# bigai-nlco/VideoTGB

Hardware: AMD Instinct MI355X
Metric: clips/sec end-to-end VideoQA (96->8 frames) (higher is better)
Workload: dtype bf16; 1 GPU; InstructBLIP-Vicuna-7B + TGB, T=96->8 of 32 frames, 224x224, greedy 16 new tokens (BASELINE.json configs[2]); inputs=resident in HBM when the timed region starts, global_batch=124, parallelism=clip-parallel x1 (no data-path collective), streams=1, weights=seeded N(0,0.02) random init

## Files before the change

include/vtgb.h:

```cpp
#ifndef VTGB_H
#define VTGB_H

#include <stddef.h>
#include <stdint.h>

#ifdef __cplusplus
extern "C" {
#endif

typedef struct ihipStream_t* vtgb_stream_t;

#define VTGB_VERSION 601

#define VTGB_OK 0
#define VTGB_EINVAL (-1)
#define VTGB_EWORKSPACE (-2)
#define VTGB_EHIP (-3)
#define VTGB_EUNSUPPORTED (-4)

#define VTGB_F32 0
#define VTGB_BF16 1
#define VTGB_BF16X3 2
#define VTGB_F16C8 3

// ... 239 lines not shown
typedef struct {
    int32_t M, N, H, W, KH, KW, C1;
    const void* a;
    const void* a2;
    const void* weights;
    const int32_t* scale;
    const float* bias;
    int32_t act;
    int32_t out_fmt;
    void* out;
    int32_t ld_out;
} vtgb_pair_conv_args;
int vtgb_pair_conv(const vtgb_pair_conv_args* a, vtgb_stream_t stream);
typedef struct {
    vtgb_pair_conv_args conv;
    const void* resid;
    int32_t ld_resid;
    const float* tail_w;
    float* tail_out;
    float* out_f32;
    int32_t ld_f32;
} vtgb_pair_conv_ex_args;
int vtgb_pair_conv_ex(const vtgb_pair_conv_ex_args* a, vtgb_stream_t stream);

typedef struct {
    int32_t dtype, n_pairs, H8, W8, dim;
    int32_t pairs_per_clip, frames_per_clip, first_off, second_off, n_images;
    float scale;
    const float* fmap;
    void* levels[4];
    void* workspace;
    size_t workspace_bytes;
} vtgb_raft_corr_args;
size_t vtgb_raft_corr_workspace_bytes(const vtgb_raft_corr_args* a);
int vtgb_raft_corr(const vtgb_raft_corr_args* a, vtgb_stream_t stream);

#define VTGB_RAFT_ENC_NW 40
typedef struct {
    int32_t dtype, n_images, H, W, norm;
    const float* images;
    const void* const* weights;
    float* out;
    void* workspace;
    size_t workspace_bytes;
} vtgb_raft_encoder_args;
size_t vtgb_raft_encoder_workspace_bytes(const vtgb_raft_encoder_args* a);
// ... 153 lines not shown
```

videotgb_amd/_lib.py:

```python
from __future__ import annotations

import ctypes as C
import os

import torch

HERE = os.path.dirname(os.path.abspath(__file__))
LIB_PATH = os.environ.get("VTGB_LIB") or os.path.join(HERE, "libvtgb.so")

F32, BF16 = 0, 1
BF16X3 = 2
F16C8 = 3
MAP_A, MAP_B = 0, 1
POOL_MEAN, POOL_CONCAT = 0, 1
TGB_MODE = {"text": 0, "vision": 0, "fusion": 1, "multi_modal": 2}
EPI_STORE, EPI_GELU, EPI_RESID_F32, EPI_STORE_F32 = 0, 1, 2, 3
VIT_NW_GLOBAL, VIT_NW_LAYER = 6, 18
QF_NW_GLOBAL, QF_NW_LAYER = 4, 32
TGB_NW_GLOBAL, TGB_NW_LAYER = 17, 26

EXPORTS = [
    "vtgb_version", "vtgb_last_error", "vtgb_pack_bf16", "vtgb_span_select", "vtgb_span_to_frames",
    "vtgb_gather_frames", "vtgb_vit_patch_kpad", "vtgb_vit_workspace_bytes", "vtgb_vit_forward",
    "vtgb_qformer_workspace_bytes", "vtgb_qformer_forward", "vtgb_pool_project_workspace_bytes",
    "vtgb_pool_project", "vtgb_tgb_workspace_bytes", "vtgb_tgb_forward", "vtgb_tgb_trunk_workspace_bytes", "vtgb_tgb_trunk",
    "vtgb_tgb_resume_workspace_bytes", "vtgb_tgb_resume", "vtgb_gemm", "vtgb_attention",
    "vtgb_layernorm", "vtgb_prof_enable", "vtgb_prof_reset", "vtgb_prof_summary", "vtgb_prof_executed_flops",
    "vtgb_llm_rmsnorm", "vtgb_llm_rope_cache", "vtgb_llm_rope_cache_prefill", "vtgb_llm_decode_attention", "vtgb_llm_silu_mul",
    "vtgb_llm_attention_rows", "vtgb_llm_gated_act", "vtgb_llm_rmsnorm_parts", "vtgb_llm_rope_cache_parts", "vtgb_gemm_skinny_splits",
    "vtgb_llm_rope_cache_pos", "vtgb_llm_rope_cache_parts_pos", "vtgb_llm_rope_cache_prefill_pos", "vtgb_llm_decode_attention_masked",
    "vtgb_llm_attention_rows_masked",
    "vtgb_gemm_skinny_workspace_bytes", "vtgb_gemm_skinny", "vtgb_pack_skinny_weight_bytes", "vtgb_pack_skinny_weight",
    "vtgb_pack_skinny_weight_fp8_bytes", "vtgb_pack_skinny_weight_fp8", "vtgb_gemm_skinny_fp8",
    "vtgb_raft_update_workspace_bytes", "vtgb_raft_update", "vtgb_raft_encoder_workspace_bytes", "vtgb_raft_encoder",
    "vtgb_raft_corr_workspace_bytes", "vtgb_raft_corr", "vtgb_preprocess_frames", "vtgb_concat_text_io", "vtgb_shifted_ce_forward", "vtgb_shifted_ce_backward",
    "vtgb_comm_unique_id", "vtgb_comm_init", "vtgb_comm_destroy", "vtgb_allreduce_f32",
    "vtgb_attn_train_forward", "vtgb_attn_train_backward",
    "vtgb_gemm_train", "vtgb_gemm_train_workspace_bytes", "vtgb_col_sum_parts", "vtgb_col_sum_f32", "vtgb_layernorm_train_partials", "vtgb_layernorm_train_forward", "vtgb_layernorm_train_backward",
    "vtgb_gelu_forward", "vtgb_gelu_backward",
    "vtgb_pair_pack", "vtgb_pair_conv", "vtgb_pair_conv_ex", "vtgb_attention_tiled",
    "vtgb_llm_decode_attention_split_workspace_bytes", "vtgb_llm_decode_attention_split",
]
COMM_ID_BYTES = 128

i32, i64, f32, vp, sz = C.c_int32, C.c_int64, C.c_float, C.c_void_p, C.c_size_t


class AttnTrainArgs(C.Structure):
    _fields_ = [("batch", i32), ("heads", i32), ("head_dim", i32), ("s_q", i32), ("s_kv", i32), ("q", vp), ("k", vp), ("v", vp),
                ("q_tok", i64), ("kv_tok", i64), ("q_batch", i64), ("kv_batch", i64), ("key_mask", vp), ("drop", vp), ("scale", f32),
                ("out", vp), ("o_tok", i64), ("o_batch", i64), ("lse", vp), ("dout", vp), ("dq", vp), ("dk", vp), ("dv", vp), ("delta", vp)]


class GemmTrainArgs(C.Structure):
    _fields_ = [("compute", i32), ("M", i32), ("N", i32), ("K", i32), ("a", vp), ("lda", i64), ("a_dtype", i32), ("a_kmajor", i32),
                ("b", vp), ("ldb", i64), ("b_dtype", i32), ("b_kmajor", i32), ("bias", vp), ("out", vp), ("ldo", i64), ("workspace", vp), ("workspace_bytes", sz)]


class LayerNormTrainArgs(C.Structure):
    _fields_ = [("rows", i32), ("D", i32), ("eps", f32), ("x", vp), ("mask", vp), ("resid", vp), ("gamma", vp), ("beta", vp), ("sum", vp),
                ("y", vp), ("mean", vp), ("rstd", vp), ("dy", vp), ("ds", vp), ("dx", vp), ("dgamma", vp), ("dbeta", vp), ("partial", vp)]


# ... 143 lines not shown
    L.vtgb_vit_patch_kpad.restype = i32
    for name, st in (("span_select", SpanSelectArgs), ("span_to_frames", SpanToFramesArgs),
                     ("gather_frames", GatherFramesArgs), ("vit_forward", VitArgs), ("qformer_forward", QFormerArgs),
                     ("pool_project", PoolProjectArgs), ("tgb_forward", TgbArgs), ("gemm", GemmArgs),
                     ("attention", AttentionArgs), ("attention_tiled", AttentionTiledArgs), ("layernorm", LayerNormArgs)):
        fn = getattr(L, "vtgb_" + name)
        fn.argtypes = [C.POINTER(st), vp]
        fn.restype = C.c_int
    for name, st in (("vit", VitArgs), ("qformer", QFormerArgs), ("pool_project", PoolProjectArgs), ("tgb", TgbArgs),
                     ("tgb_trunk", TgbSplitArgs), ("tgb_resume", TgbSplitArgs)):
        fn = getattr(L, f"vtgb_{name}_workspace_bytes")
        fn.argtypes = [C.POINTER(st)]
        fn.restype = sz
    for name in ("tgb_trunk", "tgb_resume"):
        fn = getattr(L, "vtgb_" + name)
        fn.argtypes = [C.POINTER(TgbSplitArgs), vp]
        fn.restype = C.c_int
    L.vtgb_pair_pack.argtypes = [i32, vp, vp, i64, i32, i32, vp]
    L.vtgb_pair_pack.restype = C.c_int
    L.vtgb_pair_conv.argtypes = [C.POINTER(PairConvArgs), vp]
    L.vtgb_pair_conv.restype = C.c_int
    L.vtgb_pair_conv_ex.argtypes = [C.POINTER(PairConvExArgs), vp]
    L.vtgb_pair_conv_ex.restype = C.c_int
    L.vtgb_raft_update.argtypes = [C.POINTER(RaftUpdateArgs), vp]
    L.vtgb_raft_update.restype = C.c_int
    L.vtgb_raft_update_workspace_bytes.argtypes = [C.POINTER(RaftUpdateArgs)]
    L.vtgb_raft_update_workspace_bytes.restype = sz
    L.vtgb_raft_encoder.argtypes = [C.POINTER(RaftEncoderArgs), vp]
    L.vtgb_raft_encoder.restype = C.c_int
    L.vtgb_raft_encoder_workspace_bytes.argtypes = [C.POINTER(RaftEncoderArgs)]
    L.vtgb_raft_encoder_workspace_bytes.restype = sz
    L.vtgb_raft_corr.argtypes = [C.POINTER(RaftCorrArgs), vp]
    L.vtgb_raft_corr.restype = C.c_int
    L.vtgb_raft_corr_workspace_bytes.argtypes = [C.POINTER(RaftCorrArgs)]
    L.vtgb_raft_corr_workspace_bytes.restype = sz
    L.vtgb_llm_rmsnorm.argtypes = [C.c_int, vp, vp, vp, vp, i64, i32, f32, vp]
    L.vtgb_llm_rope_cache.argtypes = [C.c_int, vp, vp, vp, vp, vp, vp, vp, i32, i32, i32, i32, i32, vp]
    L.vtgb_llm_rope_cache_prefill.argtypes = [C.c_int, vp, vp, vp, vp, vp, i32, i32, i32, i32, i32, i32, vp]
    L.vtgb_llm_decode_attention.argtypes = [C.c_int, vp, vp, vp, vp, vp, i32, i32, i32, i32, i32, f32, vp]
    L.vtgb_llm_silu_mul.argtypes = [C.c_int, vp, vp, i64, i32, vp]
    L.vtgb_llm_attention_rows.argtypes = [C.POINTER(LlmAttnRowsArgs), vp]
    L.vtgb_llm_attention_rows.restype = C.c_int
    L.vtgb_llm_gated_act.argtypes = [C.c_int, vp, vp, i64, i32, i32, i32, vp]
    L.vtgb_llm_gated_act.restype = C.c_int
    L.vtgb_llm_rmsnorm_parts.argtypes = [C.c_int, vp, vp, i32, vp, vp, i64, i32, f32, vp]
    L.vtgb_llm_rmsnorm_parts.restype = C.c_int
# ... 85 lines not shown
```

videotgb_amd/build.py:

```python
import os
import subprocess
import sys

HERE = os.path.dirname(os.path.abspath(__file__))
REPO = os.path.dirname(HERE)
CSRC = os.path.join(HERE, "csrc")
LIB = os.path.join(HERE, "libvtgb.so")
SOURCES = ["gemm.hip", "gemm_pp.hip", "gemm_h8.hip", "conv64.hip", "conv_f32.hip", "attn.hip", "attn_tiled.hip", "attn_decode.hip", "elementwise.hip", "select.hip", "forward.hip", "llm.hip", "gemm_skinny.hip", "raft.hip", "raft_x3.hip", "gru_fused.hip", "raft_corr.hip", "raft_enc.hip", "train.hip", "train_attn.hip", "train_ops.hip", "comm.hip"]


FLAGS_STAMP = os.path.join(HERE, "build", "flags")


def _flags():
    return ("debug-hooks" if os.environ.get("VTGB_DEBUG_HOOKS") == "1" else "production") + os.environ.get("VTGB_CFLAGS", "")


def _stale():
    if not os.path.exists(LIB):
        return True
    if not os.path.exists(FLAGS_STAMP) or open(FLAGS_STAMP).read() != _flags():
        return True
    t = os.path.getmtime(LIB)
    deps = [os.path.join(CSRC, f) for f in os.listdir(CSRC)] + [os.path.join(REPO, "include", "vtgb.h")]
    return any(os.path.getmtime(d) > t for d in deps)


def build(force: bool = False, verbose: bool = False) -> str:
    if not force and not _stale():
        return LIB
    hipcc = os.environ.get("HIPCC", "/opt/rocm/bin/hipcc")
# ... 31 lines not shown
```

videotgb_amd/csrc/common.h:

```cpp
#pragma once
#include <hip/hip_runtime.h>
#include <stdint.h>
#include <stdio.h>

#include "vtgb.h"

typedef __bf16 bf16_t;
typedef __attribute__((ext_vector_type(8))) __bf16 bf16x8;
typedef __attribute__((ext_vector_type(4))) __bf16 bf16x4;
typedef __attribute__((ext_vector_type(4))) float f32x4;

#if defined(__HIPCC__)
__device__ __forceinline__ float bf16_round(float v) {
    unsigned u = __float_as_uint(v);
    if ((u & 0x7F800000u) != 0x7F800000u) u += 0x7FFFu + ((u >> 16) & 1u);
    return __uint_as_float(u & 0xFFFF0000u);
}
#endif

void vtgb_set_error(const char* fmt, ...);

#define VTGB_REQUIRE(cond, code, ...)  \
    do {                               \
        if (!(cond)) {                 \
// ... 134 lines not shown
    const void *q, *k, *v;
    int64_t q_tok, kv_tok, q_batch, kv_batch;
    const float* key_mask;
    const float* rope_q;
    const float* rope_k;
    float scale;
    void* out;
    int64_t o_tok, o_batch;
    int causal = 0;
};
int launch_attention(const AttnDesc& d, hipStream_t s);

bool stem7x7_supported(int H, int W);
int launch_stem7x7(const float* img, const void* w, const float* bias, float* out_f32, float* stats, float* stats_part, void* out_bf16, int n_img, int H, int W,
                   int relu, hipStream_t s);
size_t conv64_stats_part_floats(int n_img);
int launch_stats_finish_tiles(const float* part, float* stats, int n_img, int HW, int N, int64_t M, hipStream_t s);
int launch_stats_finish_parts(const float* part, float* stats, int n_img, int parts, int C, hipStream_t s);
int cu_count();

bool conv3x3_c64_supported(int H, int W);
int launch_conv3x3_c64(const void* in, const void* w, const float* bias, float* out_f32, float* stats, float* stats_part, void* out_bf16, const void* resid,
                       int n_img, int H, int W, int relu, int post_relu, hipStream_t s);

struct LnDesc {
    int dtype, M, D;
    float eps;
    const float* x;
    int64_t ldx;
    RowMap x_map;
    const float* gamma;
    const float* beta;
    float* out_f32;
    void* out_act;
    int64_t ldo;
    RowMap o_map;
};
int launch_layernorm(const LnDesc& d, hipStream_t s);

int launch_im2col(int dtype, const float* pix, void* out, int n_img, int ch, int image, int patch, int kpad, hipStream_t s);
int launch_vit_cls_rows(const float* cls, const float* pos, float* x, int n_frames, int tokens, int hidden, hipStream_t s);
int launch_cast_act(int dtype, const float* src, void* dst, int64_t n, hipStream_t s);
int launch_mask_to_additive(const int64_t* mask, float* out, int64_t n, float neg, hipStream_t s);
int launch_fill_f32(float* dst, float v, int64_t n, hipStream_t s);
int launch_qformer_embed(const float* query, const int64_t* ids, const float* wemb, const float* pemb, float* x,
                         int n_frames, int n_query, int n_text, int hidden, hipStream_t s);
// ... 19 lines not shown
```

videotgb_amd/csrc/raft_enc.hip:

```cpp
#include <math.h>
#include <string.h>

#include "common.h"

template <typename T>
__global__ __launch_bounds__(256) void raft_stem_pack_kernel(const float* __restrict__ img, T* __restrict__ out, T* __restrict__ pad_page,
                                                             int64_t n_px, int H, int W) {
    constexpr bool PAIR = sizeof(T) == 2;
    constexpr int CP = PAIR ? 128 : 64;
    const int64_t i = (int64_t)blockIdx.x * blockDim.x + threadIdx.x;
    if (i < 64) pad_page[i] = (T)0.f;
    if (i >= n_px * 4) return;
    const int64_t px_i = i >> 2;
    const int dX = (int)(i & 3), W2 = W >> 1, H2 = H >> 1;
    const int X = (int)(px_i % W2), Y = (int)((px_i / W2) % H2);
    const int64_t n = px_i / ((int64_t)W2 * H2);
    T v[12], l[12];
#pragma unroll
    for (int py = 0; py < 2; py++)
#pragma unroll
        for (int pxx = 0; pxx < 2; pxx++) {
            const int col = 2 * (X + dX - 2) + pxx, row = 2 * Y + py;
            const bool ok = (unsigned)col < (unsigned)W;
#pragma unroll
// ... 320 lines not shown
                memset(&d, 0, sizeof(d));
                d.dtype = VTGB_BF16; d.M = (int)Mo; d.N = g.C; d.K = 9 * C2; d.epi = VTGB_EPI_STORE_F32;
                d.A = A; d.lda = C2; d.W = Wt; d.ldw = d.K; d.bias = bias; d.out = cf; d.ldo = g.Cpad;
                d.conv_H = g.Ho; d.conv_W = g.Wo; d.conv_KH = 3; d.conv_KW = 3; d.conv_Cin = C2; d.conv_split = C2; d.zero_page = zero;
                d.col_stats = col_stats; d.stats_rows = HWo;
                d.h8_run = 9 * (g.Cpad / 64); d.h8_scale = (const int*)w[40] + si;
                d.algo_flops = 2.0 * Mo * (double)g.C * (9 * g.C);
                VTGB_TRY(launch_conv_h8(d, s));
                if (col_stats) VTGB_TRY(launch_stats_finish_tiles(col_stats, stats, n, HWo, g.C, Mo, s));
                return VTGB_OK;
            };
            auto conv_pair = [&](const void* A, const void* Wt, const float* bias, int si, const void* resid, void* out, int out_bf16) -> int {
                GemmDesc d;
                memset(&d, 0, sizeof(d));
                d.dtype = VTGB_BF16; d.M = (int)Mo; d.N = g.Cpad; d.K = 9 * C2; d.epi = VTGB_EPI_SPLIT; d.act = 1;
                d.A = A; d.lda = C2; d.W = Wt; d.ldw = d.K; d.bias = bias; d.out = out; d.ldo = C2; d.split_lo = g.Cpad;
                d.conv_H = g.Ho; d.conv_W = g.Wo; d.conv_KH = 3; d.conv_KW = 3; d.conv_Cin = C2; d.conv_split = C2; d.zero_page = zero;
                d.resid_bf16 = resid; d.ldrb = C2; d.post_relu = resid != nullptr;
                d.h8_run = 9 * (g.Cpad / 64); d.h8_scale = (const int*)w[40] + si; d.h8_out_bf16 = out_bf16;
                d.algo_flops = 2.0 * Mo * (double)g.C * (9 * g.C);
                return launch_conv_h8(d, s);
            };
            const int out_h8 = (b & 1) == 0;
            if (!inorm) {
                auto split_conv = [&](int K, const void* Wt, const float* bias, int relu, void* out) -> int {
                    GemmDesc d = enc_conv(dt, (int)Mo, g.Cpad, g.Ho, g.Wo, K, Cin_pad, g.stride, Hi, Wi, x, Wt, bias, nullptr, C2, zero, nullptr);
                    d.epi = VTGB_EPI_SPLIT; d.act = relu; d.out = out; d.split_lo = g.Cpad; d.split_f16c8 = 1;
                    d.algo_flops = 2.0 * Mo * (double)g.C * (K * K * Cin_pad);
                    return launch_conv_gemm(d, s);
                };
                if (s2) VTGB_TRY(split_conv(3, bw[0], F(bw[1]), 1, t1));
                else VTGB_TRY(conv_pair(x, bw[0], F(bw[1]), 2 * b, nullptr, t1, 0));
                const void* res = x;
                outb = t2;
                if (s2) {
                    VTGB_TRY(split_conv(1, bw[4], F(bw[5]), 0, t2));
                    res = t2;
                    outb = x;
                }
                VTGB_TRY(conv_pair(t1, bw[2], F(bw[3]), 2 * b + 1, res, outb, !out_h8));
            } else {
                float* sf = stats_for(stats, HWo, g.C);
                if (s2) VTGB_TRY(conv_stats(enc_conv(dt, (int)Mo, g.C, g.Ho, g.Wo, 3, Cin_pad, g.stride, Hi, Wi, x, bw[0], F(bw[1]), cf, g.Cpad, zero, sf), stats));
                else VTGB_TRY(conv_h8(x, bw[0], F(bw[1]), sf, 2 * b));
                VTGB_TRY(norm(cf, Mo, HWo, g.C, g.Cpad, g.Cpad, nullptr, t1, 1, 0, stats, sf != nullptr, 1));
                sf = stats_for(stats, HWo, g.C);
                VTGB_TRY(conv_h8(t1, bw[2], F(bw[3]), sf, 2 * b + 1));
                const void* res = x;
                if (s2) {
                    float* sf2 = stats_for(stats2, HWo, g.C);
                    VTGB_TRY(conv_stats(enc_conv(dt, (int)Mo, g.C, g.Ho, g.Wo, 1, Cin_pad, g.stride, Hi, Wi, x, bw[4], F(bw[5]), cf2, g.Cpad, zero, sf2), stats2));
                    VTGB_TRY(norm(cf2, Mo, HWo, g.C, g.Cpad, g.Cpad, nullptr, t2, 0, 0, stats2, sf2 != nullptr));
                    res = t2;
                }
                outb = t1;
                VTGB_TRY(norm(cf, Mo, HWo, g.C, g.Cpad, g.Cpad, res, outb, 1, 1, stats, sf != nullptr, out_h8, !s2));
            }
        } else if (x3 && !inorm && g.Cpad == 128) {
            auto split_conv = [&](int K, int Cin, int stride, int Hi_, int Wi_, const void* A, const void* Wt, const float* bias, int relu, void* out) -> int {
                GemmDesc d = enc_conv(dt, (int)Mo, g.Cpad, g.Ho, g.Wo, K, Cin, stride, Hi_, Wi_, A, Wt, bias, nullptr, 2 * g.Cpad, zero, nullptr);
                d.epi = VTGB_EPI_SPLIT; d.act = relu; d.out = out; d.split_lo = g.Cpad;
                d.algo_flops = 2.0 * Mo * (double)g.C * (K * K * Cin);
                return launch_conv_gemm(d, s);
// ... 55 lines not shown
```

videotgb_amd/csrc/raft_x3.hip:

```cpp
#include <math.h>
#include <string.h>

#include "common.h"
#include "pair_h8.h"

int raft_launch_lookup_pair(const CorrPyr& pyr, const float* flow, void* out_pair, int64_t M, int H8, int W8, int h8, hipStream_t s);
int raft_lkc1_h8_pack(const void* w, void* packed, hipStream_t s);
size_t raft_lkc1_h8_pack_bytes();
int raft_launch_lookup_convc1_h8(const CorrPyr& pyr, const float* flow, const void* wpk, const int* scale, const float* bias, void* c1, int64_t M, int H8, int W8,
                                 hipStream_t s);
int raft_launch_flow_head2(const float* P2, const float* bias, float* flow, int n_pairs, int H8, int W8, hipStream_t s);
int raft_launch_upsample(const float* flow, const float* mask, float* flow_up, int n_pairs, int H8, int W8, hipStream_t s);

__device__ __forceinline__ void pair_split4(const f32x4 v, bf16x4& hi, bf16x4& lo) {
#pragma unroll
    for (int e = 0; e < 4; e++) {
        const float hf = bf16_round(v[e]);
        hi[e] = (bf16_t)hf;
        lo[e] = (bf16_t)(v[e] - hf);
    }
}
__device__ __forceinline__ f32x4 pair_join4(const bf16x4 hi, const bf16x4 lo) {
    return f32x4{(float)hi[0] + (float)lo[0], (float)hi[1] + (float)lo[1], (float)hi[2] + (float)lo[2], (float)hi[3] + (float)lo[3]};
}
// ... 341 lines not shown
        }
        if (h8) {
            GemmDesc fh = conv(256, 3, 3, hb, 128, nullptr, 0, 18, 7, F(w[19]), VTGB_EPI_SPLIT, 1, FH, 512, 256, 1);
            fh.tail_w = w[20]; fh.tail_out = P2; fh.ldtail = 32;
            VTGB_TRY(run(fh));
        } else {
            VTGB_TRY(run(conv(256, 3, 3, hb, 128, nullptr, 0, 18, 7, F(w[19]), VTGB_EPI_SPLIT, 1, FH, 512, 256, 1)));
            VTGB_TRY(launch_conv_gemm(x3_conv(Mi, 32, H8, W8, 1, 1, FH, 256, nullptr, 0, w[20], nullptr, VTGB_EPI_STORE_F32, 0, P2, 32, 0, zero), s));
        }
        VTGB_TRY(raft_launch_flow_head2(P2, F(w[21]), flow, a->n_pairs, H8, W8, s));
    }
    VTGB_TRY(run(conv(256, 3, 3, hb, 128, nullptr, 0, 22, 8, F(w[23]), VTGB_EPI_SPLIT, 1, FH, 512, 256, 1)));
    VTGB_TRY(launch_conv_gemm(x3_conv(Mi, 576, H8, W8, 1, 1, FH, 256, nullptr, 0, w[24], F(w[25]), VTGB_EPI_STORE_F32, 0, mask, 576, 0, zero), s));
    VTGB_TRY(raft_launch_upsample(flow, mask, a->flow_up, a->n_pairs, H8, W8, s));
    VTGB_HIP(hipGetLastError());
    return VTGB_OK;
}

extern "C" int vtgb_pair_pack(int32_t fmt, const float* x, void* out, int64_t M, int32_t C, int32_t ld_pair, vtgb_stream_t stream) {
    VTGB_REQUIRE(x && out && M > 0 && C > 0 && (C & 3) == 0 && ld_pair >= C && (ld_pair & 3) == 0 && (fmt == VTGB_F16C8 || fmt == VTGB_BF16X3), VTGB_EINVAL,
                 "pair_pack: bad argument (C=%d ld_pair=%d fmt=%d)", C, ld_pair, fmt);
    return launch_x3_pair_pass(x, C, nullptr, 1, nullptr, 0, 0, out, 2 * (int64_t)ld_pair, ld_pair, C, ld_pair, 0, 0, M, (hipStream_t)stream, fmt == VTGB_F16C8, 0);
}
static int pair_conv_impl(const vtgb_pair_conv_args* a, const vtgb_pair_conv_ex_args* x, vtgb_stream_t stream);
extern "C" int vtgb_pair_conv(const vtgb_pair_conv_args* a, vtgb_stream_t stream) { return pair_conv_impl(a, nullptr, stream); }
extern "C" int vtgb_pair_conv_ex(const vtgb_pair_conv_ex_args* x, vtgb_stream_t stream) {
    VTGB_REQUIRE(x, VTGB_EINVAL, "pair_conv_ex: NULL args");
    VTGB_REQUIRE((x->resid != nullptr) + (x->tail_w != nullptr) + (x->out_f32 != nullptr) <= 1, VTGB_EINVAL, "pair_conv_ex: at most one of resid / tail_w / out_f32");
    return pair_conv_impl(&x->conv, x, stream);
}
static int pair_conv_impl(const vtgb_pair_conv_args* a, const vtgb_pair_conv_ex_args* x, vtgb_stream_t stream) {
    VTGB_REQUIRE(a && a->a && a->weights && a->scale && a->out && a->M > 0 && a->N > 0 && (a->N & 1) == 0 && a->C1 > 0 && (a->C1 % 64) == 0 && a->ld_out >= a->N &&
                     (a->ld_out & 3) == 0 && (a->out_fmt == VTGB_F16C8 || a->out_fmt == VTGB_BF16X3) && (a->act == 0 || a->act == 1),
                 VTGB_EINVAL, "pair_conv: bad argument");
    static void* zero = nullptr;
    if (!zero) {
        VTGB_HIP(hipMalloc(&zero, 256));
        VTGB_HIP(hipMemset(zero, 0, 256));
    }
    GemmDesc d = h8_conv(a->M, a->N, a->H, a->W, a->KH, a->KW, a->a, a->C1, a->a2, a->a2 ? a->C1 : 0, a->weights, a->bias, VTGB_EPI_SPLIT, a->act, a->out, 2 * (int64_t)a->ld_out,
                         a->ld_out, zero, a->scale, a->out_fmt == VTGB_BF16X3);
    if (x && x->resid) {
        VTGB_REQUIRE(x->ld_resid >= a->N && (x->ld_resid & 3) == 0 && x->ld_resid == a->ld_out, VTGB_EINVAL, "pair_conv_ex: the skip operand's pair rows have the output's layout");
        d.resid_bf16 = x->resid; d.ldrb = 2 * (int64_t)x->ld_resid; d.post_relu = 1;
    }
    if (x && x->tail_w) {
        VTGB_REQUIRE(x->tail_out, VTGB_EINVAL, "pair_conv_ex: tail_out is NULL");
        d.tail_w = x->tail_w; d.tail_out = x->tail_out; d.ldtail = 32;
    }
    if (x && x->out_f32) {
        VTGB_REQUIRE(x->ld_f32 >= a->N && (x->ld_f32 & 3) == 0, VTGB_EINVAL, "pair_conv_ex: fp32 rows need ld_f32 >= N, %% 4 == 0");
        d.epi = VTGB_EPI_STORE_F32; d.out = x->out_f32; d.ldo = x->ld_f32; d.split_lo = 0;
    }
    return launch_conv_h8(d, (hipStream_t)stream);
}
```

videotgb_amd/ops.py:

```python
from __future__ import annotations

import ctypes as C
import logging
import math
from typing import Dict, List, Optional, Sequence, Tuple

import torch

from . import _lib as L
from ._lib import BF16, BF16X3, F16C8, F32

_log = logging.getLogger("videotgb_amd")
_ws_logged = set()


def _log_workspace(what: str, need: int, detail: str) -> None:
    key = (what, need >> 30)
    if key in _ws_logged:
        return
    _ws_logged.add(key)
    _log.log(logging.WARNING if need > (64 << 30) else logging.INFO, "%s: %.2f GB of workspace (%s)", what, need / 2 ** 30, detail)

Tensor = torch.Tensor

# ... 708 lines not shown
def pair_pack(x: Tensor, fmt: int = F16C8, ld_pair: Optional[int] = None) -> Tensor:
    _need_cuda(x)
    x = x.contiguous().float()
    M, Cc = x.shape
    ld = ld_pair or Cc
    out = torch.empty(M, 2 * ld, dtype=torch.int16, device=x.device)
    L.check(L.lib().vtgb_pair_pack(fmt, x.data_ptr(), out.data_ptr(), M, Cc, ld, _stream()))
    return out


def pair_unpack(rows: Tensor, C_: int, fmt: int = F16C8) -> Tensor:
    M, two_ld = rows.shape
    ld = two_ld // 2
    if fmt == BF16X3:
        v = rows.view(torch.bfloat16).float()
        return v[:, :C_] + v[:, ld:ld + C_]
    hi = rows[:, :C_].contiguous().view(torch.float16).float()
    lo = rows[:, ld:].contiguous().view(torch.uint8).reshape(M, ld // 4, 2, 4)[:, :, 0].reshape(M, ld)[:, :C_].contiguous()
    return hi + lo.view(torch.float8_e5m2).float() / H8_LO_SCALE


def pair_conv(a: Tensor, w: Tensor, sw: float, H: int, W: int, a2: Optional[Tensor] = None, bias: Optional[Tensor] = None, relu: bool = False,
              out_fmt: int = F16C8, ld_out: Optional[int] = None, resid: Optional[Tensor] = None, tail_w: Optional[Tensor] = None,
              out_f32: bool = False) -> Tensor:
    _need_cuda(a, w)
    co, kh, kw, ci = w.shape
    C1 = a.shape[1] // 2
    assert ci == C1 * (2 if a2 is not None else 1)
    _, byte = h8_weight_scale(w)
    packed = h8_conv_pack(w, sw, [C1, C1] if a2 is not None else None)
    scale = torch.tensor([byte], dtype=torch.int32, device=a.device)
    ld = ld_out or ((co + 3) // 4 * 4)
    out = torch.zeros(a.shape[0], 2 * ld, dtype=torch.int16, device=a.device)
    bias_t = None if bias is None else bias.contiguous().float()
    args = L.PairConvArgs(a.shape[0], co, H, W, kh, kw, C1, a.data_ptr(), _ptr(a2), packed.data_ptr(), scale.data_ptr(), _ptr(bias_t),
                          1 if relu else 0, out_fmt, out.data_ptr(), ld)
    if resid is None and tail_w is None and not out_f32:
        L.check(L.lib().vtgb_pair_conv(C.byref(args), _stream()))
        torch.cuda.current_stream().synchronize()
        return out
    tail_p = tail_out = f32 = None
    if tail_w is not None:
        tail_p = flow_tail_pack(tail_w.to(a.device))
        tail_out = torch.zeros(a.shape[0], 32, dtype=torch.float32, device=a.device)
    if out_f32:
        f32 = torch.zeros(a.shape[0], ld, dtype=torch.float32, device=a.device)
    ex = L.PairConvExArgs(args, _ptr(resid), ld, _ptr(tail_p), _ptr(tail_out), _ptr(f32), ld)
    L.check(L.lib().vtgb_pair_conv_ex(C.byref(ex), _stream()))
    torch.cuda.current_stream().synchronize()
    return tail_out if tail_w is not None else f32 if out_f32 else out


class RaftWeights(_WeightTable):

    def __init__(self, sd: Dict[str, Tensor], prefix: str = "update_block.", code: int = BF16, hoist_inp: Optional[bool] = None):
        super().__init__(code)
        p = prefix
        if code in (BF16X3, F16C8):
            self._init_x3(sd, p, h8=(code == F16C8))
            return
        self.hoist_inp = (code == BF16) if hoist_inp is None else (hoist_inp and code == BF16)

        def conv(name, cin_pad=None, channels=None):
            w = sd[p + name + ".weight"].float()
            if channels is not None:
                w = w[:, channels]
            co, ci, kh, kw = w.shape
            w = w.permute(0, 2, 3, 1)
            if cin_pad and cin_pad != ci:
                w = torch.nn.functional.pad(w, (0, cin_pad - ci))
            return conv_k_order(w)
# ... 275 lines not shown
```

Baseline: 37.05 clips/s.

## Add row-resident 3x3 64-channel hi/lo conv kernel for RAFT encoder residual blocks

Adds a dedicated 3x3, 64->64 channel convolution kernel over the split fp16+fp8 pair format. It keeps weights in registers, streams input rows through an LDS ring buffer via buffer-to-LDS loads, and fuses bias, ReLU, residual add and the output split. The RAFT encoder's stride-1 64-channel residual blocks and pair_conv dispatch route to it by default, replacing the generic implicit-GEMM conv path. The aim is less global memory traffic and launch overhead in the flow encoder, at the cost of a complex new kernel with possible numeric differences.

```diff
diff --git a/include/vtgb.h b/include/vtgb.h
--- a/include/vtgb.h
+++ b/include/vtgb.h
@@ -285,6 +285,8 @@
     int32_t ld_f32;
 } vtgb_pair_conv_ex_args;
 int vtgb_pair_conv_ex(const vtgb_pair_conv_ex_args* a, vtgb_stream_t stream);
+size_t vtgb_pair_conv_part_floats(int32_t n_img, int32_t H, int32_t W);
+int vtgb_pair_conv_sel(const vtgb_pair_conv_ex_args* a, int32_t kernel, float* moments, float* moments_part, vtgb_stream_t stream);
 
 typedef struct {
     int32_t dtype, n_pairs, H8, W8, dim;
diff --git a/videotgb_amd/_lib.py b/videotgb_amd/_lib.py
--- a/videotgb_amd/_lib.py
+++ b/videotgb_amd/_lib.py
@@ -38,7 +38,7 @@
     "vtgb_attn_train_forward", "vtgb_attn_train_backward",
     "vtgb_gemm_train", "vtgb_gemm_train_workspace_bytes", "vtgb_col_sum_parts", "vtgb_col_sum_f32", "vtgb_layernorm_train_partials", "vtgb_layernorm_train_forward", "vtgb_layernorm_train_backward",
     "vtgb_gelu_forward", "vtgb_gelu_backward",
-    "vtgb_pair_pack", "vtgb_pair_conv", "vtgb_pair_conv_ex", "vtgb_attention_tiled",
+    "vtgb_pair_pack", "vtgb_pair_conv", "vtgb_pair_conv_ex", "vtgb_pair_conv_sel", "vtgb_pair_conv_part_floats", "vtgb_attention_tiled",
     "vtgb_llm_decode_attention_split_workspace_bytes", "vtgb_llm_decode_attention_split",
 ]
 COMM_ID_BYTES = 128
@@ -228,6 +228,10 @@
     L.vtgb_pair_conv.restype = C.c_int
     L.vtgb_pair_conv_ex.argtypes = [C.POINTER(PairConvExArgs), vp]
     L.vtgb_pair_conv_ex.restype = C.c_int
+    L.vtgb_pair_conv_sel.argtypes = [C.POINTER(PairConvExArgs), i32, vp, vp, vp]
+    L.vtgb_pair_conv_sel.restype = C.c_int
+    L.vtgb_pair_conv_part_floats.argtypes = [i32, i32, i32]
+    L.vtgb_pair_conv_part_floats.restype = sz
     L.vtgb_raft_update.argtypes = [C.POINTER(RaftUpdateArgs), vp]
     L.vtgb_raft_update.restype = C.c_int
     L.vtgb_raft_update_workspace_bytes.argtypes = [C.POINTER(RaftUpdateArgs)]
diff --git a/videotgb_amd/build.py b/videotgb_amd/build.py
--- a/videotgb_amd/build.py
+++ b/videotgb_amd/build.py
@@ -6,7 +6,7 @@
 REPO = os.path.dirname(HERE)
 CSRC = os.path.join(HERE, "csrc")
 LIB = os.path.join(HERE, "libvtgb.so")
-SOURCES = ["gemm.hip", "gemm_pp.hip", "gemm_h8.hip", "conv64.hip", "conv_f32.hip", "attn.hip", "attn_tiled.hip", "attn_decode.hip", "elementwise.hip", "select.hip", "forward.hip", "llm.hip", "gemm_skinny.hip", "raft.hip", "raft_x3.hip", "gru_fused.hip", "raft_corr.hip", "raft_enc.hip", "train.hip", "train_attn.hip", "train_ops.hip", "comm.hip"]
+SOURCES = ["gemm.hip", "gemm_pp.hip", "gemm_h8.hip", "conv64.hip", "conv64_h8.hip", "conv_f32.hip", "attn.hip", "attn_tiled.hip", "attn_decode.hip", "elementwise.hip", "select.hip", "forward.hip", "llm.hip", "gemm_skinny.hip", "raft.hip", "raft_x3.hip", "gru_fused.hip", "raft_corr.hip", "raft_enc.hip", "train.hip", "train_attn.hip", "train_ops.hip", "comm.hip"]
 
 
 FLAGS_STAMP = os.path.join(HERE, "build", "flags")
diff --git a/videotgb_amd/csrc/common.h b/videotgb_amd/csrc/common.h
--- a/videotgb_amd/csrc/common.h
+++ b/videotgb_amd/csrc/common.h
@@ -180,6 +180,11 @@
 bool conv3x3_c64_supported(int H, int W);
 int launch_conv3x3_c64(const void* in, const void* w, const float* bias, float* out_f32, float* stats, float* stats_part, void* out_bf16, const void* resid,
                        int n_img, int H, int W, int relu, int post_relu, hipStream_t s);
+bool conv3x3_c64_h8_supported(int H, int W);
+bool conv3x3_c64_h8_enabled();
+size_t conv64_h8_stats_part_floats(int n_img, int H, int W);
+int launch_conv3x3_c64_h8(const void* in, const void* w, const int* scale, const float* bias, float* out_f32, float* stats, float* stats_part, void* out_pair,
+                          int out_bf16, const void* resid, int n_img, int H, int W, int relu, hipStream_t s);
 
 struct LnDesc {
     int dtype, M, D;
diff --git a/videotgb_amd/csrc/conv64_h8.hip b/videotgb_amd/csrc/conv64_h8.hip
--- /dev/null
+++ b/videotgb_amd/csrc/conv64_h8.hip
@@ -0,0 +1,299 @@
+#include "common.h"
+#include "pair_h8.h"
+
+namespace {
+
+constexpr int C8_R = 8, C8_RS = 64, C8_SW = C8_RS - 2;
+constexpr int C8_PLANE = C8_RS * 128;
+constexpr int C8_ROW_BYTES = 2 * C8_PLANE;
+constexpr int C8_RUN = 56;
+constexpr int C8_LDS = C8_R * C8_ROW_BYTES + 8 * 16 * 2 * 4 + 64 * 4;
+constexpr int C8_WROW = 9 * 128 * 2;
+typedef __attribute__((address_space(3))) void* c8_lptr_t;
+typedef int c8_i32x4 __attribute__((ext_vector_type(4)));
+typedef int c8_i32x8 __attribute__((ext_vector_type(8)));
+typedef _Float16 c8_f16x8 __attribute__((ext_vector_type(8)));
+constexpr int c8_vmcnt(int n) { return 0x0F70 | (n & 15) | ((n >> 4) << 14); }
+
+struct Conv64H8Params {
+    const char* in;
+    const char* w;
+    const int* scale;
+    const float* bias;
+    char* out;
+    const char* resid;
+    float* stats_part;
+    int n_img, H, W, relu;
+    int nstrips, sw, nruns;
+};
+
+template <int MODE, bool RES, int OFMT>
+__global__ __launch_bounds__(512) void conv3x3_c64_h8_kernel(const Conv64H8Params p) {
+#if defined(__HIP_DEVICE_COMPILE__)
+    extern __shared__ __attribute__((aligned(16))) char ring[];
+    float* const xch = reinterpret_cast<float*>(ring + C8_R * C8_ROW_BYTES);
+    float* const bias_s = xch + 8 * 16 * 2;
+    const int tid = threadIdx.x, lane = tid & 63, fr = lane & 15, fg = lane >> 4;
+    const int wave = __builtin_amdgcn_readfirstlane(tid >> 6);
+    const int wm = wave & 1, wn = wave >> 1;
+    const int H = p.H, W = p.W;
+    const int sc_w = *p.scale;
+
+    c8_f16x8 wf[9][2];
+    c8_i32x8 w8[9];
+    {
+        const char* const wrow = p.w + (wn * 16 + fr) * C8_WROW + fg * 16;
+#pragma unroll
+        for (int t = 0; t < 9; t++) {
+            wf[t][0] = *reinterpret_cast<const c8_f16x8*>(wrow + t * 128);
+            wf[t][1] = *reinterpret_cast<const c8_f16x8*>(wrow + t * 128 + 64);
+            w8[t].lo = *reinterpret_cast<const c8_i32x4*>(wrow + 9 * 128 + t * 128);
+            w8[t].hi = *reinterpret_cast<const c8_i32x4*>(wrow + 9 * 128 + t * 128 + 64);
+        }
+    }
+    if (tid < 64) bias_s[tid] = p.bias ? p.bias[tid] : 0.f;
+    __syncthreads();
+
+    int px[2];
+#pragma unroll
+    for (int j = 0; j < 2; j++) px[j] = wm * 32 + j * 16 + fr;
+    unsigned x_off[3];
+#pragma unroll
+    for (int kx = 0; kx < 3; kx++) x_off[kx] = (unsigned)((px[0] + kx) * 128 + ((fg ^ (((px[0] + kx) >> 1) & 7)) << 4));
+
+    typedef __attribute__((__vector_size__(4 * sizeof(unsigned)))) unsigned u32x4_t;
+    constexpr unsigned OOB = 0x80000000u;
+    constexpr int NST = MODE == 0 ? 4 : 8;
+    const unsigned ch_off = (unsigned)(wn * 16 + fg * 4) * (MODE == 0 ? 4u : 2u);
+
+    const float act_lo = p.relu ? 0.f : -__builtin_huge_valf();
+    const int per_img = p.nruns * p.nstrips, n_units = p.n_img * per_img;
+    for (int unit = blockIdx.x; unit < n_units; unit += gridDim.x) {
+        const int img = unit / per_img, ir = unit - img * per_img, run = ir / p.nstrips, strip = ir - run * p.nstrips;
+        const int xs = strip * p.sw, swd = p.sw < W - xs ? p.sw : W - xs;
+        const int y0 = run * C8_RUN, y1 = y0 + C8_RUN < H ? y0 + C8_RUN : H;
+        const int64_t ioff = (int64_t)img * H * W * 256;
+        const auto rsrc = __builtin_amdgcn_make_buffer_rsrc(const_cast<char*>(p.in + ioff), 0, H * W * 256, 0x00020000);
+        const auto orsrc = __builtin_amdgcn_make_buffer_rsrc(p.out + ioff, 0, H * W * 256, 0x00020000);
+        const auto rrsrc = __builtin_amdgcn_make_buffer_rsrc(const_cast<char*>((RES ? p.resid : p.in) + ioff), 0, H * W * 256, 0x00020000);
+        unsigned dma_off[2];
+        {
+            const int slot = wave * 8 + (lane >> 3), x = xs - 1 + slot, c = (lane & 7) ^ ((slot >> 1) & 7);
+#pragma unroll
+            for (int q = 0; q < 2; q++) dma_off[q] = (x >= 0 && x < W) ? (unsigned)(x * 256 + q * 128 + c * 16) : OOB;
+        }
+        unsigned o_off[2];
+#pragma unroll
+        for (int j = 0; j < 2; j++) o_off[j] = px[j] < swd ? (unsigned)((xs + px[j]) * 256) + ch_off : OOB;
+#define C8_ISSUE(yy)                                                                                                           \
+        {                                                                                                                      \
+            const int so_ = ((yy) >= 0 && (yy) < H) ? (yy) * W * 256 : 0x7FFFFF00;        \
+            char* const dst_ = ring + ((yy) & (C8_R - 1)) * C8_ROW_BYTES + wave * 1024;                                        \
+            __builtin_amdgcn_raw_ptr_buffer_load_lds(rsrc, (c8_lptr_t)dst_, 16, dma_off[0], so_, 0, 0);                        \
+            __builtin_amdgcn_raw_ptr_buffer_load_lds(rsrc, (c8_lptr_t)(dst_ + C8_PLANE), 16, dma_off[1], so_, 0, 0);           \
+        }
+        __builtin_amdgcn_s_waitcnt(c8_vmcnt(0));
+        __builtin_amdgcn_s_barrier();
+        C8_ISSUE(y0 - 1)
+        C8_ISSUE(y0)
+        C8_ISSUE(y0 + 1)
+        C8_ISSUE(y0 + 2)
+        f32x4 s1 = {0.f, 0.f, 0.f, 0.f}, s2 = s1;
+        for (int y = y0; y < y1; y += 2) {
+            if (y == y0) __builtin_amdgcn_s_waitcnt(c8_vmcnt(0));
+            else __builtin_amdgcn_s_waitcnt(c8_vmcnt(NST));
+            __builtin_amdgcn_s_barrier();
+            h8_u32x2 rh[2][2], rl[2][2];
+            if constexpr (RES) {
+#pragma unroll
+                for (int o = 0; o < 2; o++)
+#pragma unroll
+                    for (int j = 0; j < 2; j++) {
+                        const unsigned off = (y + o < y1 && o_off[j] != OOB) ? o_off[j] + (unsigned)((y + o) * W * 256) : OOB;
+                        rh[o][j] = __builtin_amdgcn_raw_buffer_load_b64(rrsrc, off, 0, 0);
+                        rl[o][j] = __builtin_amdgcn_raw_buffer_load_b64(rrsrc, off + 128u, 0, 0);
+                    }
+            }
+            C8_ISSUE(y + 3)
+            C8_ISSUE(y + 4)
+            const f32x4 b4 = *reinterpret_cast<const f32x4*>(bias_s + wn * 16 + fg * 4);
+            f32x4 acc[2][2];
+#pragma unroll
+            for (int o = 0; o < 2; o++)
+#pragma unroll
+                for (int j = 0; j < 2; j++) acc[o][j] = b4;
+#pragma unroll
+            for (int rr = 0; rr < 4; rr++) {
+                const char* const rowp = ring + ((y + rr - 1) & (C8_R - 1)) * C8_ROW_BYTES;
+#pragma unroll
+                for (int kx = 0; kx < 3; kx++) {
+                    c8_f16x8 xa[2][2];
+#pragma unroll
+                    for (int j = 0; j < 2; j++) {
+                        xa[j][0] = *reinterpret_cast<const c8_f16x8*>(rowp + x_off[kx] + j * 2048);
+                        xa[j][1] = *reinterpret_cast<const c8_f16x8*>(rowp + (x_off[kx] ^ 64u) + j * 2048);
+                    }
+#pragma unroll
+                    for (int part = 0; part < 2; part++)
+#pragma unroll
+                        for (int o = 0; o < 2; o++) {
+                            const int ky = rr - o;
+                            if (ky < 0 || ky > 2) continue;
+#pragma unroll
+                            for (int j = 0; j < 2; j++)
+                                acc[o][j] = __builtin_amdgcn_mfma_f32_16x16x32_f16(wf[ky * 3 + kx][part], xa[j][part], acc[o][j], 0, 0, 0);
+                        }
+                }
+                __builtin_amdgcn_sched_barrier(0);
+            }
+            __builtin_amdgcn_sched_barrier(0);
+#pragma unroll
+            for (int rr = 0; rr < 4; rr++) {
+                const char* const rowp = ring + ((y + rr - 1) & (C8_R - 1)) * C8_ROW_BYTES + C8_PLANE;
+#pragma unroll
+                for (int kx = 0; kx < 3; kx++) {
+                    c8_i32x8 xc[2];
+#pragma unroll
+                    for (int j = 0; j < 2; j++) {
+                        xc[j].lo = *reinterpret_cast<const c8_i32x4*>(rowp + x_off[kx] + j * 2048);
+                        xc[j].hi = *reinterpret_cast<const c8_i32x4*>(rowp + (x_off[kx] ^ 64u) + j * 2048);
+                    }
+#pragma unroll
+                    for (int o = 0; o < 2; o++) {
+                        const int ky = rr - o;
+                        if (ky < 0 || ky > 2) continue;
+#pragma unroll
+                        for (int j = 0; j < 2; j++)
+                            acc[o][j] = __builtin_amdgcn_mfma_scale_f32_16x16x128_f8f6f4(w8[ky * 3 + kx], xc[j], acc[o][j], 0, 1, 0, sc_w, 0, 127);
+                    }
+                }
+                __builtin_amdgcn_sched_barrier(0);
+            }
+#pragma unroll
+            for (int o = 0; o < 2; o++) {
+                const bool row_ok = y + o < y1;
+#pragma unroll
+                for (int j = 0; j < 2; j++) {
+                    const bool ok = row_ok && o_off[j] != OOB;
+                    const unsigned off = ok ? o_off[j] + (unsigned)((y + o) * W * 256) : OOB;
+                    f32x4 v = acc[o][j];
+                    if constexpr (MODE == 0) {
+                        __builtin_amdgcn_raw_buffer_store_b128(__builtin_bit_cast(u32x4_t, v), orsrc, off, 0, 0);
+                        const f32x4 vz = {ok ? v[0] : 0.f, ok ? v[1] : 0.f, ok ? v[2] : 0.f, ok ? v[3] : 0.f};
+                        s1 += vz;
+                        s2 += vz * vz;
+                    } else {
+                        v = f32x4{fmaxf(v[0], act_lo), fmaxf(v[1], act_lo), fmaxf(v[2], act_lo), fmaxf(v[3], act_lo)};
+                        if constexpr (RES) {
+                            v += h8_join4(rh[o][j], rl[o][j]);
+                            v = f32x4{fmaxf(v[0], 0.f), fmaxf(v[1], 0.f), fmaxf(v[2], 0.f), fmaxf(v[3], 0.f)};
+                        }
+                        h8_u32x2 hu, lu;
+                        if constexpr (OFMT == 1) {
+                            h8_split4(v, hu, lu);
+                        } else {
+                            const f32x4 hf = {bf16_round(v[0]), bf16_round(v[1]), bf16_round(v[2]), bf16_round(v[3])};
+                            const bf16x4 hi = {(bf16_t)hf[0], (bf16_t)hf[1], (bf16_t)hf[2], (bf16_t)hf[3]};
+                            const bf16x4 lo = {(bf16_t)(v[0] - hf[0]), (bf16_t)(v[1] - hf[1]), (bf16_t)(v[2] - hf[2]), (bf16_t)(v[3] - hf[3])};
+                            hu = __builtin_bit_cast(h8_u32x2, hi); lu = __builtin_bit_cast(h8_u32x2, lo);
+                        }
+                        __builtin_amdgcn_raw_buffer_store_b64(hu, orsrc, off, 0, 0);
+                        __builtin_amdgcn_raw_buffer_store_b64(lu, orsrc, ok ? off + 128u : OOB, 0, 0);
+                    }
+                }
+            }
+        }
+#undef C8_ISSUE
+        if constexpr (MODE == 0) {
+#pragma unroll
+            for (int e = 0; e < 4; e++) {
+                float a_ = s1[e], b_ = s2[e];
+#pragma unroll
+                for (int off = 1; off < 16; off <<= 1) { a_ += __shfl_xor(a_, off); b_ += __shfl_xor(b_, off); }
+                s1[e] = a_; s2[e] = b_;
+            }
+            __builtin_amdgcn_s_waitcnt(0xC07F);
+            __builtin_amdgcn_s_barrier();
+            if (fr == 0) {
+#pragma unroll
+                for (int e = 0; e < 4; e++) {
+                    xch[(wave * 16 + fg * 4 + e) * 2] = s1[e];
+                    xch[(wave * 16 + fg * 4 + e) * 2 + 1] = s2[e];
+                }
+            }
+            __syncthreads();
+            if (tid < 128 && p.stats_part) {
+                const int ch = tid >> 1, which = tid & 1, wn_ = ch >> 4, c16 = ch & 15;
+                const float t = xch[((wn_ * 2) * 16 + c16) * 2 + which] + xch[((wn_ * 2 + 1) * 16 + c16) * 2 + which];
+                p.stats_part[((int64_t)unit * 64 + ch) * 2 + which] = t;
+            }
+        }
+    }
+#endif
+}
+
+static void c8_geometry(int H, int W, int& nstrips, int& sw, int& nruns) {
+    nstrips = (W + C8_SW - 1) / C8_SW;
+    sw = (W + nstrips - 1) / nstrips;
+    nruns = (H + C8_RUN - 1) / C8_RUN;
+}
+
+}
+
+bool conv3x3_c64_h8_supported(int H, int W) { return W >= 4 && W <= 2 * C8_SW && H >= 1 && (int64_t)H * W * 256 < 0x7FFFFF00ll; }
+
+bool conv3x3_c64_h8_enabled() {
+#ifdef VTGB_DEBUG_HOOKS
+    static const bool on = !(getenv("VTGB_CONV64_H8") && getenv("VTGB_CONV64_H8")[0] == '0');
+    return on;
+#else
+    return true;
+#endif
+}
+
+size_t conv64_h8_stats_part_floats(int n_img, int H, int W) {
+    int nstrips, sw, nruns;
+    c8_geometry(H, W, nstrips, sw, nruns);
+    return (size_t)n_img * nstrips * nruns * 64 * 2;
+}
+
+int launch_conv3x3_c64_h8(const void* in, const void* w, const int* scale, const float* bias, float* out_f32, float* stats, float* stats_part, void* out_pair,
+                          int out_bf16, const void* resid, int n_img, int H, int W, int relu, hipStream_t s) {
+    VTGB_REQUIRE(conv3x3_c64_h8_supported(H, W), VTGB_EUNSUPPORTED, "conv3x3_c64_h8: %d x %d outside W in [4, %d]", H, W, 2 * C8_SW);
+    VTGB_REQUIRE(in && w && scale && (out_f32 || out_pair) && n_img > 0, VTGB_EINVAL, "conv3x3_c64_h8: NULL operand");
+    Conv64H8Params p;
+    p.in = (const char*)in; p.w = (const char*)w; p.scale = scale; p.bias = bias; p.out = out_f32 ? (char*)out_f32 : (char*)out_pair; p.resid = (const char*)resid;
+    p.stats_part = stats ? stats_part : nullptr; p.n_img = n_img; p.H = H; p.W = W; p.relu = relu;
+    c8_geometry(H, W, p.nstrips, p.sw, p.nruns);
+    const int64_t units = (int64_t)n_img * p.nstrips * p.nruns;
+    VTGB_REQUIRE(units < (1ll << 31), VTGB_EUNSUPPORTED, "conv3x3_c64_h8: too many work units");
+    const int grid = units < cu_count() ? (int)units : cu_count();
+    const double flops = 2.0 * n_img * H * W * 64.0 * 576.0;
+    ProfScope prof(VTGB_PROF_CONV, flops, s, 2.0 * flops);
+    static DeviceOnce a0, a10, a11, a20, a21;
+    if (out_f32) {
+        VTGB_REQUIRE(!stats || stats_part, VTGB_EINVAL, "conv3x3_c64_h8: partial-moment scratch missing");
+        VTGB_REQUIRE(!resid && !relu, VTGB_EUNSUPPORTED, "conv3x3_c64_h8: fp32 rows come without activation or skip");
+        VTGB_FUNC_LDS_ONCE(a0, (conv3x3_c64_h8_kernel<0, false, 1>), C8_LDS);
+        hipLaunchKernelGGL((conv3x3_c64_h8_kernel<0, false, 1>), dim3(grid), dim3(512), C8_LDS, s, p);
+        if (stats) VTGB_TRY(launch_stats_finish_parts(stats_part, stats, n_img, p.nstrips * p.nruns, 64, s));
+    } else if (!resid) {
+        if (out_bf16) {
+            VTGB_FUNC_LDS_ONCE(a10, (conv3x3_c64_h8_kernel<1, false, 0>), C8_LDS);
+            hipLaunchKernelGGL((conv3x3_c64_h8_kernel<1, false, 0>), dim3(grid), dim3(512), C8_LDS, s, p);
+        } else {
+            VTGB_FUNC_LDS_ONCE(a11, (conv3x3_c64_h8_kernel<1, false, 1>), C8_LDS);
+            hipLaunchKernelGGL((conv3x3_c64_h8_kernel<1, false, 1>), dim3(grid), dim3(512), C8_LDS, s, p);
+        }
+    } else {
+        if (out_bf16) {
+            VTGB_FUNC_LDS_ONCE(a20, (conv3x3_c64_h8_kernel<1, true, 0>), C8_LDS);
+            hipLaunchKernelGGL((conv3x3_c64_h8_kernel<1, true, 0>), dim3(grid), dim3(512), C8_LDS, s, p);
+        } else {
+            VTGB_FUNC_LDS_ONCE(a21, (conv3x3_c64_h8_kernel<1, true, 1>), C8_LDS);
+            hipLaunchKernelGGL((conv3x3_c64_h8_kernel<1, true, 1>), dim3(grid), dim3(512), C8_LDS, s, p);
+        }
+    }
+    VTGB_HIP(hipGetLastError());
+    return VTGB_OK;
+}
diff --git a/videotgb_amd/csrc/raft_enc.hip b/videotgb_amd/csrc/raft_enc.hip
--- a/videotgb_amd/csrc/raft_enc.hip
+++ b/videotgb_amd/csrc/raft_enc.hip
@@ -366,6 +366,8 @@
                 return launch_conv_h8(d, s);
             };
             const int out_h8 = (b & 1) == 0;
+            const bool c64h = conv3x3_c64_h8_enabled() && g.C == 64 && g.Cpad == 64 && Cin_pad == 64 && !s2 && conv3x3_c64_h8_supported(g.Ho, g.Wo);
+            const int* const hs = (const int*)w[40];
             if (!inorm) {
                 auto split_conv = [&](int K, const void* Wt, const float* bias, int relu, void* out) -> int {
                     GemmDesc d = enc_conv(dt, (int)Mo, g.Cpad, g.Ho, g.Wo, K, Cin_pad, g.stride, Hi, Wi, x, Wt, bias, nullptr, C2, zero, nullptr);
@@ -374,6 +376,7 @@
                     return launch_conv_gemm(d, s);
                 };
                 if (s2) VTGB_TRY(split_conv(3, bw[0], F(bw[1]), 1, t1));
+                else if (c64h) VTGB_TRY(launch_conv3x3_c64_h8(x, bw[0], hs + 2 * b, F(bw[1]), nullptr, nullptr, nullptr, t1, 0, nullptr, n, g.Ho, g.Wo, 1, s));
                 else VTGB_TRY(conv_pair(x, bw[0], F(bw[1]), 2 * b, nullptr, t1, 0));
                 const void* res = x;
                 outb = t2;
@@ -382,7 +385,8 @@
                     res = t2;
                     outb = x;
                 }
-                VTGB_TRY(conv_pair(t1, bw[2], F(bw[3]), 2 * b + 1, res, outb, !out_h8));
+                if (c64h) VTGB_TRY(launch_conv3x3_c64_h8(t1, bw[2], hs + 2 * b + 1, F(bw[3]), nullptr, nullptr, nullptr, outb, !out_h8, res, n, g.Ho, g.Wo, 1, s));
+                else VTGB_TRY(conv_pair(t1, bw[2], F(bw[3]), 2 * b + 1, res, outb, !out_h8));
             } else {
                 float* sf = stats_for(stats, HWo, g.C);
                 if (s2) VTGB_TRY(conv_stats(enc_conv(dt, (int)Mo, g.C, g.Ho, g.Wo, 3, Cin_pad, g.stride, Hi, Wi, x, bw[0], F(bw[1]), cf, g.Cpad, zero, sf), stats));
diff --git a/videotgb_amd/csrc/raft_x3.hip b/videotgb_amd/csrc/raft_x3.hip
--- a/videotgb_amd/csrc/raft_x3.hip
+++ b/videotgb_amd/csrc/raft_x3.hip
@@ -387,17 +387,38 @@
                  "pair_pack: bad argument (C=%d ld_pair=%d fmt=%d)", C, ld_pair, fmt);
     return launch_x3_pair_pass(x, C, nullptr, 1, nullptr, 0, 0, out, 2 * (int64_t)ld_pair, ld_pair, C, ld_pair, 0, 0, M, (hipStream_t)stream, fmt == VTGB_F16C8, 0);
 }
-static int pair_conv_impl(const vtgb_pair_conv_args* a, const vtgb_pair_conv_ex_args* x, vtgb_stream_t stream);
+static int pair_conv_impl(const vtgb_pair_conv_args* a, const vtgb_pair_conv_ex_args* x, vtgb_stream_t stream, int kernel = 0, float* moments = nullptr,
+                          float* moments_part = nullptr);
 extern "C" int vtgb_pair_conv(const vtgb_pair_conv_args* a, vtgb_stream_t stream) { return pair_conv_impl(a, nullptr, stream); }
+extern "C" size_t vtgb_pair_conv_part_floats(int32_t n_img, int32_t H, int32_t W) {
+    return n_img > 0 && conv3x3_c64_h8_supported(H, W) ? conv64_h8_stats_part_floats(n_img, H, W) : 0;
+}
+extern "C" int vtgb_pair_conv_sel(const vtgb_pair_conv_ex_args* x, int32_t kernel, float* moments, float* moments_part, vtgb_stream_t stream) {
+    VTGB_REQUIRE(x && kernel >= 0 && kernel <= 2, VTGB_EINVAL, "pair_conv_sel: NULL args or kernel %d outside 0..2", kernel);
+    VTGB_REQUIRE((x->resid != nullptr) + (x->tail_w != nullptr) + (x->out_f32 != nullptr) <= 1, VTGB_EINVAL, "pair_conv_sel: at most one of resid / tail_w / out_f32");
+    VTGB_REQUIRE(!moments || (x->out_f32 && moments_part), VTGB_EINVAL, "pair_conv_sel: moments come with out_f32 and need moments_part");
+    return pair_conv_impl(&x->conv, x, stream, kernel, moments, moments_part);
+}
 extern "C" int vtgb_pair_conv_ex(const vtgb_pair_conv_ex_args* x, vtgb_stream_t stream) {
     VTGB_REQUIRE(x, VTGB_EINVAL, "pair_conv_ex: NULL args");
     VTGB_REQUIRE((x->resid != nullptr) + (x->tail_w != nullptr) + (x->out_f32 != nullptr) <= 1, VTGB_EINVAL, "pair_conv_ex: at most one of resid / tail_w / out_f32");
     return pair_conv_impl(&x->conv, x, stream);
 }
-static int pair_conv_impl(const vtgb_pair_conv_args* a, const vtgb_pair_conv_ex_args* x, vtgb_stream_t stream) {
+static int pair_conv_impl(const vtgb_pair_conv_args* a, const vtgb_pair_conv_ex_args* x, vtgb_stream_t stream, int kernel, float* moments, float* moments_part) {
     VTGB_REQUIRE(a && a->a && a->weights && a->scale && a->out && a->M > 0 && a->N > 0 && (a->N & 1) == 0 && a->C1 > 0 && (a->C1 % 64) == 0 && a->ld_out >= a->N &&
                      (a->ld_out & 3) == 0 && (a->out_fmt == VTGB_F16C8 || a->out_fmt == VTGB_BF16X3) && (a->act == 0 || a->act == 1),
                  VTGB_EINVAL, "pair_conv: bad argument");
+    {
+        const bool f32 = x && x->out_f32;
+        const bool fits = a->KH == 3 && a->KW == 3 && a->C1 == 64 && a->N == 64 && !a->a2 && !(x && x->tail_w) && a->H > 0 && a->W > 0 && a->M % (a->H * a->W) == 0 &&
+                          (f32 ? x->ld_f32 == 64 && a->act == 0 : a->ld_out == 64) && (!(x && x->resid) || x->ld_resid == 64) && conv3x3_c64_h8_supported(a->H, a->W);
+        VTGB_REQUIRE(kernel != 2 || fits, VTGB_EUNSUPPORTED, "pair_conv_sel: the row-resident kernel takes 3x3, 64 -> 64 channels, 64-unit rows, W <= 124");
+        const bool take = kernel == 2 || (kernel == 0 && fits && conv3x3_c64_h8_enabled());
+        VTGB_REQUIRE(!moments || take, VTGB_EUNSUPPORTED, "pair_conv_sel: moments come from the row-resident kernel only");
+        if (take)
+            return launch_conv3x3_c64_h8(a->a, a->weights, a->scale, a->bias, f32 ? x->out_f32 : nullptr, moments, moments_part, f32 ? nullptr : a->out,
+                                         a->out_fmt == VTGB_BF16X3, x ? x->resid : nullptr, a->M / (a->H * a->W), a->H, a->W, a->act, (hipStream_t)stream);
+    }
     static void* zero = nullptr;
     if (!zero) {
         VTGB_HIP(hipMalloc(&zero, 256));
diff --git a/videotgb_amd/ops.py b/videotgb_amd/ops.py
--- a/videotgb_amd/ops.py
+++ b/videotgb_amd/ops.py
@@ -754,7 +754,7 @@
 
 def pair_conv(a: Tensor, w: Tensor, sw: float, H: int, W: int, a2: Optional[Tensor] = None, bias: Optional[Tensor] = None, relu: bool = False,
               out_fmt: int = F16C8, ld_out: Optional[int] = None, resid: Optional[Tensor] = None, tail_w: Optional[Tensor] = None,
-              out_f32: bool = False) -> Tensor:
+              out_f32: bool = False, kernel: int = 0, moments: bool = False):
     _need_cuda(a, w)
     co, kh, kw, ci = w.shape
     C1 = a.shape[1] // 2
@@ -767,7 +767,7 @@
     bias_t = None if bias is None else bias.contiguous().float()
     args = L.PairConvArgs(a.shape[0], co, H, W, kh, kw, C1, a.data_ptr(), _ptr(a2), packed.data_ptr(), scale.data_ptr(), _ptr(bias_t),
                           1 if relu else 0, out_fmt, out.data_ptr(), ld)
-    if resid is None and tail_w is None and not out_f32:
+    if resid is None and tail_w is None and not out_f32 and kernel == 0:
         L.check(L.lib().vtgb_pair_conv(C.byref(args), _stream()))
         torch.cuda.current_stream().synchronize()
         return out
@@ -778,7 +778,18 @@
     if out_f32:
         f32 = torch.zeros(a.shape[0], ld, dtype=torch.float32, device=a.device)
     ex = L.PairConvExArgs(args, _ptr(resid), ld, _ptr(tail_p), _ptr(tail_out), _ptr(f32), ld)
-    L.check(L.lib().vtgb_pair_conv_ex(C.byref(ex), _stream()))
+    if kernel == 0 and not moments:
+        L.check(L.lib().vtgb_pair_conv_ex(C.byref(ex), _stream()))
+    else:
+        mom = part = None
+        if moments:
+            n_img = a.shape[0] // (H * W)
+            mom = torch.zeros(n_img, 64, 2, dtype=torch.float32, device=a.device)
+            part = torch.zeros(max(1, L.lib().vtgb_pair_conv_part_floats(n_img, H, W)), dtype=torch.float32, device=a.device)
+        L.check(L.lib().vtgb_pair_conv_sel(C.byref(ex), kernel, _ptr(mom), _ptr(part), _stream()))
+        if moments:
+            torch.cuda.current_stream().synchronize()
+            return f32, mom
     torch.cuda.current_stream().synchronize()
     return tail_out if tail_w is not None else f32 if out_f32 else out
 
```

After: 37.33 clips/s, median of 6. Within noise of the previous version (+0.7%).
